# lucidrains/nuwa-pytorch

Hardware: AMD Instinct MI355X
Metric: video-tokens/sec, 3DNA decoder fwd+bwd @ 10x16x16 (higher is better)
Workload: dtype bf16/fp16 operands, fp32 accumulate -- forward: 3-MFMA bf16 hi+lo pairs on cross-attention kv projection, to_logits; 2 fp16 MFMAs (fp16 activation x fp16 hi+lo weight) on to_out x2, cross-attention q projection; single fp16 MFMA on 3DNA q/k/v projection, FF1 + gate, FF2, Sparse3DNA core, cross-atten

## Files before the change

### nuwa_pytorch_amd/csrc/s3_args.h

```cpp
#pragma once
#include <type_traits>
#include "common.h"
#include "../../include/amdnuwa.h"

struct S3Args {
    const bf16_t *q, *k, *v, *ql, *kl, *vl; int ld;
    bf16_t *o, *ol; int ldo;
    int ol_f16;
    const bf16_t *dO, *dOl; int lddo;
    bf16_t *dq, *dk, *dv, *dql, *dkl, *dvl; int ldd;
    const float* wth;
    const float* bias;
    float *ds, *pm;
    float* stats;
    float *part_th, *part_k0, *part_v0;
    float* dwth;
    int B, ntok, F, H, W, kf, kh, kw, df, dh, dw, NH;
    int of, oh, ow;
    int xmode, FK, kvrows, kvoff, ldk, lddk;
    const bf16_t *k0, *k0l, *v0, *v0l; long long k0_bs;
    const uint8_t* kmask;
    float *dnull_k, *dnull_v;
    float scale;
    int accumulate;
    int dbg;
    int ymajor;
    int sep_passes;
    int packed;
    const float* gs2;
    int NT, TW, SW;
};

struct S3DropArgs : S3Args { const uint8_t* keep; float drop_s; };
template <bool DROP> struct S3KArgsSel { using type = S3Args; };
template <> struct S3KArgsSel<true> { using type = S3DropArgs; };
template <bool DROP> using S3KArgs = typename S3KArgsSel<DROP>::type;
template <bool DROP> inline S3KArgs<DROP> s3_kargs(const S3Args& a, const uint8_t* keep, float drop_s) {
    if constexpr (DROP) {
        S3DropArgs d{};
        static_cast<S3Args&>(d) = a;
        d.keep = keep; d.drop_s = drop_s;
        return d;
    } else {
        return a;
    }
}

struct S3Tile { int tw, nt, sw; };
// ... 108 lines not shown
```

### nuwa_pytorch_amd/csrc/sparse3dna.hip

```cpp
#include <cmath>
#include "common.h"
#include "s3_args.h"

namespace {

constexpr int KHMAX = 3;

struct PlaneIt { int ta, tb, fr, yr; };

template <int CH, typename Fn>
__device__ __forceinline__ void sweep_taps(const S3Args& a, const bf16_t* src, const bf16_t* srcl, int b, int f, int y, int w,
                                           int h, int c, bool act, bool qvalid, bf16_t* st_hi, Fn&& fn) {
    const int HS = a.W * a.NH * 32;
    bf16_t* st_lo = st_hi + (CH / 8) * HS;
    const int myslot = ((w * a.NH + h) * 4 + c) * 8;
    const int yr0 = y - a.oh * a.dh;
    uint4 rh[CH / 8], rl[CH / 8];
    auto seek = [&](PlaneIt& p) {
        while (p.ta < a.kf && !(p.fr >= 0 && p.yr >= 0 && p.fr < a.FK && p.yr < a.H)) {
            ++p.tb; p.yr += a.dh;
            if (p.tb == a.kh) { p.tb = 0; p.yr = yr0; ++p.ta; p.fr += a.df; }
        }
    };
    auto step = [&](PlaneIt& p) {
// ... 490 lines not shown
                else {
                    const size_t ci = (((size_t)b * nq + pq) * J + 1 + slot_plane(tp) * a.kw + tc) * a.NH + h;
                    dsv = a.ds[ci]; pmv = a.pm[ci];
                }
                const int slot = ((wq * a.NH + h) * 4 + c) * 8;
                if (LO) {
                    float qq[CH], dd[CH];
                    load_chunk<CH>(sq_hi + slot, a.ql ? sq_lo + slot : nullptr, qq, HS);
                    load_chunk<CH>(sd_hi + slot, a.dOl ? sd_lo + slot : nullptr, dd, HS);
#pragma unroll
                    for (int e = 0; e < CH; ++e) { dkf[e] += dsv * qq[e]; dvf[e] += pmv * dd[e]; }
                } else {
                    uint32_t qk2[CH / 2], dk2[CH / 2];
                    load_pk<CH>(sq_hi + slot, qk2, HS);
                    load_pk<CH>(sd_hi + slot, dk2, HS);
                    axpy_pk<CH>(dkf, dsv, qk2);
                    axpy_pk<CH>(dvf, pmv, dk2);
                }
            }
        }
        tp = tn;
    }
    if (kvalid) {
#pragma unroll
        for (int e = 0; e < CH; ++e) dkf[e] *= a.scale;
        const size_t g = ((size_t)b * a.kvrows + ik) * a.lddk + h * DH + c * CH;
        store_chunk<CH>(a.dk + g, a.dkl ? a.dkl + g : nullptr, dkf);
        store_chunk<CH>(a.dv + g, a.dvl ? a.dvl + g : nullptr, dvf);
    }
}

__global__ __launch_bounds__(1024) void s3_bwd_fin_kernel(S3Args a, int DH) {
    __shared__ float red[2][16][64];
    const int rows = a.F * a.H * a.NT, inner = a.NH * DH;
    const int lane = threadIdx.x & 63, rg = threadIdx.x >> 6;
    const int nchunk = (inner + 63) / 64;
    if ((int)blockIdx.x >= a.B * nchunk) {
        __shared__ float redw[64][17];
        const int nn = a.NH * a.NH;
        const int col = (blockIdx.x - a.B * nchunk) * 16 + (threadIdx.x & 15), rg64 = threadIdx.x >> 4;
        float s = 0.f;
        if (col < nn) {
            const int n = a.B * rows;
            for (int k = rg64; k < n; k += 64 * 8) {
                float v[8];
#pragma unroll
                for (int u = 0; u < 8; ++u) {
                    const int ku = k + 64 * u;
                    const float t = a.part_th[(size_t)(ku < n ? ku : 0) * nn + col];
                    v[u] = ku < n ? t : 0.f;
                }
#pragma unroll
                for (int u = 0; u < 8; ++u) s += v[u];
            }
        }
        redw[rg64][threadIdx.x & 15] = s;
        __syncthreads();
        if (rg64 == 0 && col < nn) {
            float t = 0.f;
#pragma unroll
            for (int r = 0; r < 64; ++r) t += redw[r][threadIdx.x & 15];
            t *= f16_gs_inv(a.gs2);
            a.dwth[col] = a.accumulate ? a.dwth[col] + t : t;
        }
        return;
    }
    if (a.xmode) {
// ... 116 lines not shown
        y = cl + (ii / a.F) * a.dh; f = ii % a.F;
        return;
    }
    y = r2 / a.F; f = r2 % a.F;
}
constexpr int S3M_PAD = 4;
__device__ __forceinline__ int s3m_ts(int J) { return J * S3M_NH + S3M_PAD; }
__device__ __forceinline__ int s3m_item(int item, float rJ) { return item * S3M_NH + (int)(((float)item + 0.5f) * rJ) * S3M_PAD; }

#ifndef S3_MIX_PIN
#define S3_MIX_PIN 0
#endif
#if S3_MIX_PIN
#define S3_MIX_PIN_ASM(s) asm volatile("" : "+v"(s))
#else
#define S3_MIX_PIN_ASM(s) ((void)0)
#endif
__device__ __forceinline__ void lds_store8_done(float* p, const float (&v)[8]) {
#if S3_MIX_PIN
    __builtin_amdgcn_sched_barrier(0);
#endif
#pragma unroll
    for (int g = 0; g < 8; ++g) p[g] = v[g];
#if S3_MIX_PIN
    asm volatile("s_waitcnt lgkmcnt(0)" ::: "memory");
    __builtin_amdgcn_sched_barrier(0);
#endif
}

__device__ __forceinline__ uint2 s3m_keep8(const uint8_t* keep, size_t item) { return *reinterpret_cast<const uint2*>(keep + item * S3M_NH); }
__device__ __forceinline__ bool s3m_kept(uint2 m, int g) { return (((g < 4 ? m.x : m.y) >> (8 * (g & 3))) & 0xffu) != 0u; }
__device__ __forceinline__ bool s3m_kept(uint32_t m, int g) { return ((m >> (8 * g)) & 0xffu) != 0u; }

__device__ __forceinline__ void rowm_planes(const S3Args& a, int f, int y, int* pslot, int* ptok) {
    const int ta0 = max(0, a.kf - 1 - f / a.df), tb0 = max(0, a.kh - 1 - y / a.dh);
    const int nb = a.kh - tb0, n = (a.kf - ta0) * nb;
    const int e = threadIdx.x;
    if (e < n) {
        const int ta = ta0 + e / nb, tb = tb0 + e % nb;
        pslot[e] = 1 + (ta * a.kh + tb) * a.kw;
        ptok[e] = 1 + ((f - (a.kf - 1 - ta) * a.df) * a.H + (y - (a.kh - 1 - tb) * a.dh)) * S3M_W;
    }
    if (e == 0) pslot[S3M_PLANES] = n;
    __syncthreads();
}
__device__ __forceinline__ RowM rowm_init(const S3Args& a, int b, int ry, const int* pslot, const int* ptok) {
    RowM r;
    r.nplanes = pslot[S3M_PLANES];
    r.J = a.kf * a.kh * a.kw + 1;
    r.TS = s3m_ts(r.J);
    r.lane = threadIdx.x & 63; r.wave = threadIdx.x >> 6; r.c = r.lane & 15; r.g4 = r.lane >> 4;
    r.tok0 = (size_t)b * a.ntok;
    r.iq = 1 + ry * S3M_W + r.c;
    r.qok = r.iq < a.ntok;
    r.pslot = pslot; r.ptok = ptok;
    r.vps = r.lane < r.nplanes ? pslot[r.lane] : 0;
    r.vpt = r.lane < r.nplanes ? ptok[r.lane] : 0;
#pragma unroll
    for (int q = 0; q < 4; ++q) {
        const int d = r.c - (4 * r.g4 + q);
        r.tsel[q] = -1;
#pragma unroll
        for (int tc = 0; tc < S3M_KW; ++tc)
            if (tc < a.kw && d == (a.kw - 1 - tc) * a.dw) r.tsel[q] = tc;
    }
    return r;
}

__device__ __forceinline__ void mfma_band_scores(const S3Args& a, const RowM& r, const bf16_t* rows, int ldr, const bf16_t* frag,
                                                 int ldf, int h, float* TAB, float mul, const float* bias) {
    constexpr int NH = S3M_NH, DH = S3M_DH;
    const bf16_t* qrow = frag + (r.tok0 + r.iq) * ldf + h * DH + r.g4 * 8;
    const bf16x8 qf0 = ldg8(qrow, r.qok), qf1 = ldg8(qrow + 32, r.qok);
    const bf16_t* kbase = rows + r.tok0 * ldr + h * DH + r.g4 * 8;
    const int spb = r.c * r.TS + h;
    int sidx[4];
#pragma unroll
    for (int q = 0; q < 4; ++q) sidx[q] = spb + (r.tsel[q] < 0 ? 0 : r.tsel[q]) * NH;
    constexpr int PF = S3M_PF;
    bf16x8 kq0[PF], kq1[PF];
    auto issue = [&](int sq, bf16x8& d0, bf16x8& d1) {
        if (sq > r.nplanes) { d0 = d1 = bf16x8{}; return; }
        const int tok = sq == 0 ? 0 : r.ptok[sq - 1] + r.c;
        const bf16_t* kp = kbase + (size_t)tok * ldr;
// ... 275 lines not shown
            d0 = base + r8 < a.ntok ? ldg_u4(sb, so + v0) : make_uint4(0, 0, 0, 0);
            d1 = base + r8 + 8 < a.ntok ? ldg_u4(sb, so + v1) : make_uint4(0, 0, 0, 0);
        }
    };
    fetch2(0, st[0], st[1]); fetch2(1, st[2], st[3]);
    for (int pi = 0; pi < r.nplanes; pi += 2) {
#pragma unroll
        for (int i = 0; i < 4; ++i) *reinterpret_cast<uint4*>(tile + woff[i]) = st[i];
        const unsigned jb0 = 4u * NH * (unsigned)__builtin_amdgcn_readlane(r.vps, pi);
        const bool two = pi + 1 < r.nplanes;
        const unsigned jb1 = two ? 4u * NH * (unsigned)__builtin_amdgcn_readlane(r.vps, pi + 1) : jb0;
        if (pi + 2 < r.nplanes) { fetch2(pi + 2, st[0], st[1]); fetch2(pi + 3, st[2], st[3]); }
        float pf[8];
#pragma unroll
        for (int j = 0; j < 4; ++j) {
            const float x0 = lds_ld32(sidx4[j] + jb0), x1 = lds_ld32(sidx4[j] + jb1);
            pf[j] = on[j] ? x0 : 0.f;
            pf[4 + j] = (on[j] && two) ? x1 : 0.f;
        }
        const bf16x8 pb = __builtin_bit_cast(bf16x8, make_uint4(pack2_t<F16>(pf[0], pf[1]), pack2_t<F16>(pf[2], pf[3]),
                                                                 pack2_t<F16>(pf[4], pf[5]), pack2_t<F16>(pf[6], pf[7])));
        __builtin_amdgcn_wave_barrier();
#pragma unroll
        for (int db = 0; db < 4; ++db) {
            const s16x4 lo = __builtin_amdgcn_ds_read_tr16_b64_v4i16((lds_s16x4_t*)(tile + troff[db]));
            const s16x4 hi = __builtin_amdgcn_ds_read_tr16_b64_v4i16((lds_s16x4_t*)(tile + troff[db] + 2048));
            const s16x8 v8 = {lo[0], lo[1], lo[2], lo[3], hi[0], hi[1], hi[2], hi[3]};
            O[db] = mfma16<F16>(__builtin_bit_cast(bf16x8, v8), pb, O[db]);
        }
        __builtin_amdgcn_wave_barrier();
    }
}

__device__ __forceinline__ void rowm_softmax(float* TAB, int J, float* gst = nullptr, int wvalid = 0, float pre = 1.f) {
    constexpr int NH = S3M_NH;
    const int t = threadIdx.x, cc = t & 3, wh = t >> 2, h = wh % NH, w = wh / NH;
    TAB += w * s3m_ts(J) + h;
    if (J <= 48) {
        float v[12];
#pragma unroll
        for (int k = 0; k < 12; ++k) { const int j = cc + 4 * k; v[k] = j < J ? TAB[j * NH] * pre : NEG_MAX; }
        float m = NEG_MAX;
#pragma unroll
        for (int k = 0; k < 12; ++k) m = fmaxf(m, v[k]);
        m = quad_max(m);
        float sum = 0.f;
#pragma unroll
        for (int k = 0; k < 12; ++k) {
            const float e = cc + 4 * k < J ? __expf(v[k] - m) : 0.f;
            v[k] = e;
            if (cc + 4 * k < J) sum += e;
        }
        sum = quad_sum(sum);
        const float inv = 1.f / sum;
#pragma unroll
        for (int k = 0; k < 12; ++k) { const int j = cc + 4 * k; if (j < J) TAB[j * NH] = v[k] * inv; }
        if (gst && cc == 0 && w < wvalid) *reinterpret_cast<float2*>(gst + (w * NH + h) * 4) = make_float2(m, inv);
        return;
    }
    float m = NEG_MAX;
    for (int j = cc; j < J; j += 4) m = fmaxf(m, TAB[j * NH] * pre);
    m = quad_max(m);
    float sum = 0.f;
    for (int j = cc; j < J; j += 4) {
        const int idx = j * NH;
        const float e = __expf(TAB[idx] * pre - m);
        TAB[idx] = e;
        sum += e;
    }
// ... 579 lines not shown
    __syncthreads();
    {
        const int g = r.wave;
        f32x4 O[ROWS][4];
        if (!(a.dbg & 4)) {
            if (r.nk <= 64) tile_band_apply_fast<ROWS, F16>(a, r, a.v, a.ld, g, SP, vt_base + r.wave * 4096, O);
            else tile_band_apply<ROWS, F16>(a, r, a.v, a.ld, g, SP, vt_base + r.wave * 4096, O);
        }
        else {
#pragma unroll
            for (int i = 0; i < ROWS; ++i)
#pragma unroll
                for (int db = 0; db < 4; ++db) O[i][db] = f32x4{0.f, 0.f, 0.f, 0.f};
        }
#pragma unroll
        for (int i = 0; i < ROWS; ++i) {
            if (!r.qok[i]) continue;
            const size_t go = (r.tok0 + r.iq[i]) * a.ldo + g * DH + 4 * r.g4;
#pragma unroll
            for (int db = 0; db < 4; ++db) {
                const uint32_t h01 = pack2_rne(O[i][db][0], O[i][db][1]), h23 = pack2_rne(O[i][db][2], O[i][db][3]);
                if (!F16 || a.o) *reinterpret_cast<uint2*>(a.o + go + db * 16) = make_uint2(h01, h23);
                if (F16 && a.ol)
                    *reinterpret_cast<uint2*>(a.ol + go + db * 16) = a.ol_f16 ?
                        make_uint2(pack2_f16_sat(O[i][db][0], O[i][db][1]), pack2_f16_sat(O[i][db][2], O[i][db][3])) :
                        make_uint2(pack2_rne(O[i][db][0] - lo_f(h01), O[i][db][1] - hi_f(h01)), pack2_rne(O[i][db][2] - lo_f(h23), O[i][db][3] - hi_f(h23)));
            }
        }
    }
}

typedef _Float16 f16x4_t __attribute__((ext_vector_type(4)));
constexpr float S3Q_DPS = 0.015625f;
template <bool BIAS, bool G16 = false, bool DROP = false>
__global__ __launch_bounds__(512, 4) void s3_bwd_q_mfma_kernel(S3KArgs<DROP> a) {
    constexpr int NH = S3M_NH, DH = S3M_DH, W = S3M_W, inner = NH * DH;
    extern __shared__ __attribute__((aligned(16))) char smem[];
    const int J = a.kf * a.kh * a.kw + 1, TS = s3m_ts(J), nsp = W * TS;
    const float rJ = 1.f / (float)J;
    const size_t r1 = (size_t)nsp * 4 > 8 * 4096 ? (size_t)nsp * 4 : 8 * 4096;
    float* SP = reinterpret_cast<float*>(smem);
    float* DP = reinterpret_cast<float*>(smem + r1);
    float* RED = DP + nsp;
    float* PM0 = RED + 8 * 64;
    __shared__ float wsh[64];
    __shared__ int pslot[S3M_PLANES + 1], ptok[S3M_PLANES + 1];
    const int t = threadIdx.x;
    const int rows = a.F * a.H;
    const int bid = xcd_row_id();
    const int b = bid / rows, r2 = bid % rows;
    int f, y;
    s3m_row_order(a, r2, f, y);
    const int ry = f * a.H + y;
    const int nq = a.ntok - 1;
    if (t < NH * NH) wsh[t] = a.wth[t];
    float* pth = a.part_th + (size_t)bid * NH * NH;
    float* pk0 = a.part_k0 + (size_t)bid * inner;
    float* pv0 = a.part_v0 + (size_t)bid * inner;
    if (ry == 0)
        for (int e = t; e < inner; e += blockDim.x) a.dq[((size_t)b * a.ntok) * a.ldd + e] = 0;
    if (ry * W + 1 >= a.ntok) {
        for (int e = t; e < NH * NH; e += blockDim.x) pth[e] = 0.f;
        for (int e = t; e < inner; e += blockDim.x) { pk0[e] = 0.f; pv0[e] = 0.f; }
        return;
    }
    {
        const float4 neg4 = make_float4(NEG_MAX, NEG_MAX, NEG_MAX, NEG_MAX), zero4 = make_float4(0.f, 0.f, 0.f, 0.f);
        for (int e = t; e < nsp / 4 && !(a.dbg & 2048); e += blockDim.x) { reinterpret_cast<float4*>(SP)[e] = neg4; reinterpret_cast<float4*>(DP)[e] = zero4; }
    }
    rowm_planes(a, f, y, pslot, ptok);
    const RowM r = rowm_init(a, b, ry, pslot, ptok);
    char* stile = reinterpret_cast<char*>(PM0 + W * NH) + r.wave * 2048;
    if (!(a.dbg & 1)) {
    if constexpr (!BIAS) {
    mfma_band_scores_fast<G16>(a, r, a.k, a.ld, a.q, a.ld, r.wave, SP, 1.f, stile);
    mfma_band_scores_fast<G16>(a, r, a.v, a.ld, a.dO, a.lddo, r.wave, DP, G16 ? S3Q_DPS : 1.f, stile);
    } else {
    mfma_band_scores_staged<G16>(a, r, a.k, a.ld, a.q, a.ld, r.wave, SP, BIAS ? a.scale : 1.f, BIAS ? a.bias : nullptr, stile);
    mfma_band_scores_staged<G16>(a, r, a.v, a.ld, a.dO, a.lddo, r.wave, DP, G16 ? S3Q_DPS : 1.f, nullptr, stile);
    }
    }
    __syncthreads();
    float* gst = a.stats ? a.stats + ((size_t)b * nq + (size_t)ry * W) * NH * 4 : nullptr;
    const int wvalid = a.ntok - 1 - ry * W;
    if (!(a.dbg & 64)) rowm_softmax(SP, J, gst, wvalid, BIAS ? 1.f : a.scale);
    [[maybe_unused]] float dps_back = 1.f / S3Q_DPS;
    if constexpr (DROP) {
        dps_back *= a.drop_s;
        const float sdp = G16 ? 1.f : a.drop_s;
        for (int item = t; item < W * J; item += blockDim.x) {
            const int wq = (int)(((float)item + 0.5f) * rJ), iq = 1 + ry * W + wq;
            if (iq < a.ntok) {
                const uint2 m = s3m_keep8(a.keep, ((size_t)b * nq + (iq - 1)) * J + (item - wq * J));
                const int ib = item * NH + wq * S3M_PAD;
                float4 d0 = *reinterpret_cast<const float4*>(DP + ib), d1 = *reinterpret_cast<const float4*>(DP + ib + 4);
                d0.x = s3m_kept(m, 0) ? d0.x * sdp : 0.f; d0.y = s3m_kept(m, 1) ? d0.y * sdp : 0.f;
                d0.z = s3m_kept(m, 2) ? d0.z * sdp : 0.f; d0.w = s3m_kept(m, 3) ? d0.w * sdp : 0.f;
                d1.x = s3m_kept(m, 4) ? d1.x * sdp : 0.f; d1.y = s3m_kept(m, 5) ? d1.y * sdp : 0.f;
                d1.z = s3m_kept(m, 6) ? d1.z * sdp : 0.f; d1.w = s3m_kept(m, 7) ? d1.w * sdp : 0.f;
                *reinterpret_cast<float4*>(DP + ib) = d0;
                *reinterpret_cast<float4*>(DP + ib + 4) = d1;
            }
        }
    }
    __syncthreads();
    if constexpr (G16) {
        const int lane = t & 63, wv = t >> 6, n16 = lane & 15, kg = lane >> 4, sset = n16 >> 3, kh = kg & 1;
        const bool on = (n16 < 8) == (kg < 2);
        f16x4_t awt_hi, awt_lo;
#pragma unroll
        for (int i = 0; i < 4; ++i) {
            const float wt = on ? wsh[(4 * kh + i) * NH + (n16 & 7)] : 0.f;
            const _Float16 h16 = (_Float16)wt;
            awt_hi[i] = h16; awt_lo[i] = (_Float16)(wt - (float)h16);
        }
        const int nitems = W * J, ngrp = (nitems + 31) >> 5;
        f32x4 CW = {0.f, 0.f, 0.f, 0.f};
        float dp_amax = 0.f;
        for (int G = wv; G < ngrp && !(a.dbg & 128); G += 8) {
            {
                const int ib0 = 32 * G + 16 * sset + 4 * kg;
                float avf[4], bvf[4];
#pragma unroll
                for (int ts = 0; ts < 4; ++ts) {
                    const int item = ib0 + ((ts + sset + 2 * kh) & 3);
                    const bool ok = item < nitems;
                    const int idx = s3m_item(ok ? item : 0, rJ) + (n16 & 7);
                    avf[ts] = ok ? DP[idx] : 0.f;
                    bvf[ts] = ok ? SP[idx] : 0.f;
                }
                const f16x4_t av = __builtin_bit_cast(f16x4_t, make_uint2(pack2_f16_sat(avf[0], avf[1]), pack2_f16_sat(avf[2], avf[3])));
                const f16x4_t bv = __builtin_bit_cast(f16x4_t, make_uint2(pack2_f16(bvf[0], bvf[1]), pack2_f16(bvf[2], bvf[3])));
                CW = __builtin_amdgcn_mfma_f32_16x16x16f16(av, bv, CW, 0, 0, 0);
            }
            const int item = 32 * G + 16 * (kg >> 1) + n16;
            const bool ok = item < nitems;
            const int ib = s3m_item(ok ? item : 0, rJ) + 4 * kh;
            const float4 d4 = *reinterpret_cast<const float4*>(DP + ib);
            const f16x4_t df = __builtin_bit_cast(f16x4_t, make_uint2(pack2_f16_sat_n(d4.x, d4.y, dp_amax), pack2_f16_sat_n(d4.z, d4.w, dp_amax)));
            f32x4 rr = {0.f, 0.f, 0.f, 0.f};
            rr = __builtin_amdgcn_mfma_f32_16x16x16f16(awt_hi, df, rr, 0, 0, 0);
            rr = __builtin_amdgcn_mfma_f32_16x16x16f16(awt_lo, df, rr, 0, 0, 0);
            if (ok) *reinterpret_cast<float4*>(DP + ib) = make_float4(rr[0], rr[1], rr[2], rr[3]);
        }
        f16_sat_commit(dp_amax);
        float tw[4];
#pragma unroll
        for (int i = 0; i < 4; ++i) tw[i] = CW[i] + __shfl(CW[i], (lane + 40) & 63, 64);
        if (n16 < 8 && kg < 2) {
#pragma unroll
            for (int i = 0; i < 4; ++i) RED[wv * 64 + (4 * kg + i) * NH + n16] = tw[i] * dps_back;
        }
        __syncthreads();
        if (t < NH * NH) {
            float sum = 0.f;
            for (int k = 0; k < 8; ++k) sum += RED[k * 64 + t];
            pth[t] = sum;
        }
        __syncthreads();
    } else if (!a.sep_passes) {
        float red_lane = 0.f;
#pragma unroll
        for (int half = 0; half < 2; ++half) {
            float acc[32];
#pragma unroll
            for (int k = 0; k < 32; ++k) acc[k] = 0.f;
#pragma unroll 1
            for (int item = t; item < W * J && !(a.dbg & 128); item += blockDim.x) {
                const int wq = (int)(((float)item + 0.5f) * rJ), j = item - wq * J;
                const int iq = 1 + ry * W + wq;
                const int ib = item * NH + wq * S3M_PAD;
                const float4 p0 = *reinterpret_cast<const float4*>(SP + ib), p1 = *reinterpret_cast<const float4*>(SP + ib + 4);
                const float4 d0 = *reinterpret_cast<const float4*>(DP + ib), d1 = *reinterpret_cast<const float4*>(DP + ib + 4);
                const float pv[8] = {p0.x, p0.y, p0.z, p0.w, p1.x, p1.y, p1.z, p1.w};
                const float dv_[8] = {d0.x, d0.y, d0.z, d0.w, d1.x, d1.y, d1.z, d1.w};
                const float* wv = wsh;
                asm volatile("" : "+v"(wv));
                float res[8];
#pragma unroll
                for (int x = 0; x < 8; ++x) res[x] = 0.f;
#pragma unroll
                for (int g = 0; g < 8; ++g) {
                    const float4 w0 = *reinterpret_cast<const float4*>(wv + g * NH), w1 = *reinterpret_cast<const float4*>(wv + g * NH + 4);
                    const float wg[8] = {w0.x, w0.y, w0.z, w0.w, w1.x, w1.y, w1.z, w1.w};
                    if (half == 0) {
                        if (!a.packed) {
                            float sm = 0.f;
#pragma unroll
                            for (int hh = 0; hh < 8; ++hh) sm += wg[hh] * pv[hh];
                            res[g] = sm;
                        }
// ... 8 lines not shown
                }
                if (half == 0) {
                    if (!a.packed) {
                        if constexpr (DROP) {
                            if (iq < a.ntok) {
                                const uint2 m = s3m_keep8(a.keep, ((size_t)b * nq + (iq - 1)) * J + j);
#pragma unroll
                                for (int g = 0; g < 8; ++g) res[g] = s3m_kept(m, g) ? res[g] * a.drop_s : 0.f;
                            }
                        }
                        if (iq < a.ntok && !gst && !(a.dbg & 2)) {
                            float4* dst = reinterpret_cast<float4*>(a.pm + (((size_t)b * nq + (iq - 1)) * J + j) * NH);
                            dst[0] = make_float4(res[0], res[1], res[2], res[3]);
                            dst[1] = make_float4(res[4], res[5], res[6], res[7]);
                        }
                        if (j == 0) {
#pragma unroll
                            for (int g = 0; g < 8; ++g) PM0[wq * NH + g] = iq < a.ntok ? res[g] : 0.f;
                        }
                    }
                } else {
                    *reinterpret_cast<float4*>(DP + ib) = make_float4(res[0], res[1], res[2], res[3]);
                    *reinterpret_cast<float4*>(DP + ib + 4) = make_float4(res[4], res[5], res[6], res[7]);
                }
            }
            const int lane = t & 63;
#pragma unroll
            for (int off = 16, cnt = 16; off >= 1; off >>= 1, cnt >>= 1) {
                const bool upper = (lane & off) != 0;
#pragma unroll
                for (int i = 0; i < cnt; ++i) {
                    const float send = upper ? acc[i] : acc[i + cnt];
                    const float keep = upper ? acc[i + cnt] : acc[i];
                    acc[i] = keep + __shfl_xor(send, off, 64);
                }
            }
            const float tot = acc[0] + __shfl_xor(acc[0], 32, 64);
            if ((lane >> 5) == half) red_lane = tot;
        }
        RED[(t >> 6) * 64 + (t & 63)] = red_lane;
        __syncthreads();
        if (t < NH * NH) {
            float s = 0.f;
            for (int k = 0; k < 8; ++k) s += RED[k * 64 + t];
            pth[t] = s;
        }
        __syncthreads();
    } else {
        float wr[64];
#pragma unroll
        for (int k = 0; k < 64; ++k) wr[k] = wsh[k];
        for (int item0 = t; item0 < (gst ? W : W * J); item0 += blockDim.x) {
            const int item = gst ? item0 * J : item0;
            const int wq = (int)(((float)item + 0.5f) * rJ), j = item - wq * J;
            const int iq = 1 + ry * W + wq;
            float pv[8];
    #pragma unroll
            for (int hh = 0; hh < 8; ++hh) pv[hh] = SP[item * NH + wq * S3M_PAD + hh];
            float* dst = a.pm + (((size_t)b * nq + (iq - 1)) * J + j) * NH;
            [[maybe_unused]] uint2 km = make_uint2(0u, 0u);
            if constexpr (DROP) { if (iq < a.ntok) km = s3m_keep8(a.keep, ((size_t)b * nq + (iq - 1)) * J + j); }
    #pragma unroll
            for (int g = 0; g < 8; ++g) {
                float s = 0.f;
    #pragma unroll
                for (int hh = 0; hh < 8; ++hh) s += wr[g * NH + hh] * pv[hh];
                if constexpr (DROP) s = s3m_kept(km, g) ? s * a.drop_s : 0.f;
                if (iq < a.ntok && !gst && !(a.dbg & 2)) dst[g] = s;
                if (j == 0) PM0[wq * NH + g] = iq < a.ntok ? s : 0.f;
            }
        }
        {
            const int pair = t & 63, grp = t >> 6;
            const int g = pair / NH, hh = pair % NH;
            float acc = 0.f;
            for (int item = grp; item < W * J && !(a.dbg & 8); item += 8 * 8) {
                float dv8[8], pv8[8];
    #pragma unroll
                for (int u = 0; u < 8; ++u) {
                    const int it = item + 8 * u, itc = it < W * J ? it : grp;
                    const int ib = s3m_item(itc, rJ);
                    dv8[u] = DP[ib + g]; pv8[u] = SP[ib + hh];
                }
    #pragma unroll
                for (int u = 0; u < 8; ++u) acc += item + 8 * u < W * J ? dv8[u] * pv8[u] : 0.f;
            }
            RED[grp * 64 + pair] = acc;
            __syncthreads();
            if (t < NH * NH) {
                float s = 0.f;
                for (int k = 0; k < 8; ++k) s += RED[k * 64 + t];
                pth[t] = s;
            }
            __syncthreads();
        }
        for (int item = t; item < W * J; item += blockDim.x) {
            float dv_[8], out[8];
            const int ib = s3m_item(item, rJ);
    #pragma unroll
            for (int g = 0; g < 8; ++g) dv_[g] = DP[ib + g];
    #pragma unroll
            for (int hh = 0; hh < 8; ++hh) {
                float s = 0.f;
    #pragma unroll
                for (int g = 0; g < 8; ++g) s += wr[g * NH + hh] * dv_[g];
                S3_MIX_PIN_ASM(s);
                out[hh] = s;
            }
            lds_store8_done(DP + ib, out);
        }
        __syncthreads();
    }
    {
        const int cc = t & 3, wh = t >> 2, h = wh % NH, w = wh / NH;
        const int i = 1 + ry * W + w;
        float ds_amax = 0.f;
        if (a.dbg & 256) {
        } else if (J <= 48) {
            float pv[12], dv[12];
#pragma unroll
            for (int k = 0; k < 12; ++k) {
                const int j = cc + 4 * k, idx = w * TS + (j < J ? j : cc) * NH + h;
                pv[k] = SP[idx]; dv[k] = DP[idx];
            }
            float d = 0.f;
#pragma unroll
            for (int k = 0; k < 12; ++k) if (cc + 4 * k < J) d += pv[k] * dv[k];
            d = quad_sum(d);
            if (gst && cc == 0 && i < a.ntok) gst[(w * NH + h) * 4 + 2] = d;
#pragma unroll
            for (int k = 0; k < 12; ++k) {
                const int j = cc + 4 * k;
                if (j < J) {
                    const int idx = w * TS + j * NH + h;
                    float dsv = pv[k] * (dv[k] - d);
                    if constexpr (G16) { dsv *= dps_back; ds_amax = fmaxf(ds_amax, fabsf(dsv)); dsv = f16_clamp(dsv); }
                    DP[idx] = dsv;
                    if (i < a.ntok && !gst && !a.packed && !(a.dbg & 2)) a.ds[(((size_t)b * nq + (i - 1)) * J + j) * NH + h] = dsv;
                }
            }
        } else {
        float d = 0.f;
        for (int j = cc; j < J; j += 4) d += SP[w * TS + j * NH + h] * DP[w * TS + j * NH + h];
        d = quad_sum(d);
// ... 119 lines not shown
        const int eg = t & 63, wv = t >> 6, h = eg >> 3;
        float sk[8], sv[8];
#pragma unroll
        for (int k = 0; k < 8; ++k) { sk[k] = 0.f; sv[k] = 0.f; }
        uint4 qv[2], dv4[2];
        float cs[2], cp[2];
#pragma unroll
        for (int rr = 0; rr < 2; ++rr) {
            const int w = 2 * wv + rr, i = 1 + ry * W + w;
            const bool in = i < a.ntok;
            const size_t ic = r.tok0 + (in ? i : a.ntok - 1);
            qv[rr] = *reinterpret_cast<const uint4*>(a.q + ic * a.ld + 8 * eg);
            dv4[rr] = *reinterpret_cast<const uint4*>(a.dO + ic * a.lddo + 8 * eg);
            cs[rr] = in ? DP[w * TS + h] : 0.f;
            cp[rr] = in ? PM0[w * NH + h] : 0.f;
        }
#pragma unroll
        for (int rr = 0; rr < 2; ++rr) {
            const uint32_t qw[4] = {qv[rr].x, qv[rr].y, qv[rr].z, qv[rr].w}, dw[4] = {dv4[rr].x, dv4[rr].y, dv4[rr].z, dv4[rr].w};
#pragma unroll
            for (int k = 0; k < 4; ++k) {
                sk[2 * k] = fmaf(cs[rr], lo_t<G16>(qw[k]), sk[2 * k]); sk[2 * k + 1] = fmaf(cs[rr], hi_t<G16>(qw[k]), sk[2 * k + 1]);
                sv[2 * k] = fmaf(cp[rr], lo_t<G16>(dw[k]), sv[2 * k]); sv[2 * k + 1] = fmaf(cp[rr], hi_t<G16>(dw[k]), sv[2 * k + 1]);
            }
        }
        float4* dst = reinterpret_cast<float4*>(part + (wv * 64 + eg) * 16);
        const int rot = eg >> 2;
        dst[rot & 3] = make_float4(sk[0], sk[1], sk[2], sk[3]); dst[(1 + rot) & 3] = make_float4(sk[4], sk[5], sk[6], sk[7]);
        dst[(2 + rot) & 3] = make_float4(sv[0], sv[1], sv[2], sv[3]); dst[(3 + rot) & 3] = make_float4(sv[4], sv[5], sv[6], sv[7]);
    }
    __syncthreads();
    if (!(a.dbg & 1024)) {
        const float* part = reinterpret_cast<const float*>(smem);
        for (int e = t; e < inner; e += blockDim.x) {
            const int eg = e >> 3, cmp = e & 7, rot = eg >> 2;
            const int ok_ = 4 * (((cmp >> 2) + rot) & 3) + (cmp & 3), ov_ = 4 * ((2 + (cmp >> 2) + rot) & 3) + (cmp & 3);
            float sk = 0.f, sv = 0.f;
#pragma unroll
            for (int wv = 0; wv < 8; ++wv) {
                sk += part[(wv * 64 + eg) * 16 + ok_];
                sv += part[(wv * 64 + eg) * 16 + ov_];
            }
            pk0[e] = a.scale * sk;
            pv0[e] = sv;
        }
    }
}

template <bool PACKED, bool G16 = false>
__global__ __launch_bounds__(512, 2) void s3_bwd_kv_mfma_kernel(S3Args a) {
    constexpr int NH = S3M_NH, DH = S3M_DH, W = S3M_W;
    extern __shared__ __attribute__((aligned(16))) char smem[];
    __shared__ int pslot[S3M_PLANES + 1], ptok[S3M_PLANES + 1];
    const int t = threadIdx.x, lane = t & 63, wave = t >> 6, c = lane & 15, g4 = lane >> 4, h = wave;
    const int rows = a.F * a.H;
    const int bid = xcd_row_id();
    const int b = bid / rows, r2 = bid % rows;
    int f, y;
    s3m_row_order(a, r2, f, y);
    const int ry = f * a.H + y;
    const int J = a.kf * a.kh * a.kw + 1, nq = a.ntok - 1;
    if (ry * W + 1 >= a.ntok) return;
    if (t < 64) {
        const int ta = t / a.kh, tb = t % a.kh;
        const int fq = f + (a.kf - 1 - ta) * a.df, yq = y + (a.kh - 1 - tb) * a.dh;
        const bool ok = t < a.kf * a.kh && fq < a.F && yq < a.H && (fq * a.H + yq) * W + 1 < a.ntok;
        const unsigned long long m = __ballot(ok);
        if (ok) {
            const int pos = __popcll(m & ((1ull << t) - 1ull));
            pslot[pos] = 1 + (ta * a.kh + tb) * a.kw; ptok[pos] = 1 + (fq * a.H + yq) * W;
        }
        if (t == 0) pslot[S3M_PLANES] = __popcll(m);
    }
    __syncthreads();
    const int nplanes = pslot[S3M_PLANES];
    const size_t tok0 = (size_t)b * a.ntok;
    int tsel[4];
#pragma unroll
    for (int j = 0; j < 4; ++j) {
// ... 304 lines not shown
        __builtin_amdgcn_wave_barrier();
    }
    if (kok) {
        bf16_t* kr = a.dk + (tok0 + ik) * a.ldd + h * DH + 4 * g4;
        bf16_t* vr = a.dv + (tok0 + ik) * a.ldd + h * DH + 4 * g4;
        float amax = 0.f;
#pragma unroll
        for (int db = 0; db < 4; ++db) {
            if constexpr (G16) {
                *reinterpret_cast<uint2*>(kr + db * 16) = make_uint2(pack2_f16_sat_n(dK[db][0] * a.scale, dK[db][1] * a.scale, amax),
                                                                     pack2_f16_sat_n(dK[db][2] * a.scale, dK[db][3] * a.scale, amax));
                *reinterpret_cast<uint2*>(vr + db * 16) = make_uint2(pack2_f16_sat_n(dV[db][0], dV[db][1], amax), pack2_f16_sat_n(dV[db][2], dV[db][3], amax));
            } else {
                *reinterpret_cast<uint2*>(kr + db * 16) = make_uint2(pack2_rne(dK[db][0] * a.scale, dK[db][1] * a.scale),
                                                                     pack2_rne(dK[db][2] * a.scale, dK[db][3] * a.scale));
                *reinterpret_cast<uint2*>(vr + db * 16) = make_uint2(pack2_rne(dV[db][0], dV[db][1]), pack2_rne(dV[db][2], dV[db][3]));
            }
        }
        if constexpr (G16) f16_sat_commit(amax);
    }
}


bool s3_mfma_geom(const amdnuwa_s3_geom* g) {
    return !g->noncausal && g->W == 16 && g->heads == 8 && g->dim_head == 64 && g->kw <= S3M_KW && g->kf * g->kh <= S3M_PLANES;
}
int s3_tile_rows(const amdnuwa_s3_geom* g, int want) {
    if (want == 0) want = S3T_AUTO_ROWS;
    for (int rws = want >= 4 ? 4 : (want >= 2 ? 2 : 1); rws > 1; rws >>= 1)
        if (g->dh > 0 && g->H % (g->dh * rws) == 0 && g->kf * (g->kh + rws - 1) <= S3T_MAXK) return rws;
    return 1;
}

enum : int { S3K_FWD = 3,
             S3K_BWD = 4,
             S3K_TILE_ROWS = 16,
             S3K_SEP_PASSES = 19,
             S3K_WS_FP32 = 24,
             S3K_DROP_VALU = 26 };
enum S3Form { S3_BF16, S3_HILO, S3_F16 };
enum S3KvSide { S3KV_VALU, S3KV_BAND_F32, S3KV_BAND_PACKED, S3KV_BAND_RC };
struct S3Route {
    bool f16;
    bool fwd_band; int tile_rows;
    bool q_band; S3KvSide kv;
    int packed, sep_passes, ymajor;
};
S3Route s3_route(const amdnuwa_s3_geom* g, S3Form form, bool masked, bool cross = false) {
    const int* t = g_amdnuwa_tuning;
    S3Route r{};
    r.tile_rows = 1;
    r.ymajor = (t[S3K_FWD] & 2) ? 0 : 1;
    if (cross) return r;
    if (form == S3_F16) {
        r.f16 = r.fwd_band = r.q_band = true; r.kv = S3KV_BAND_PACKED; r.packed = 1;
    } else {
        const bool band = form == S3_BF16 && s3_mfma_geom(g) && !(masked && t[S3K_DROP_VALU] == 1);
        r.fwd_band = band && !(t[S3K_FWD] & 1);
        r.q_band = band && t[S3K_BWD] != 1;
        const bool kv_band = r.q_band && t[S3K_BWD] != 2;
        r.sep_passes = t[S3K_SEP_PASSES] == 1;
        r.packed = (kv_band && !g->d_rel_bias && t[S3K_WS_FP32] != 1 && !r.sep_passes) ? 1 : 0;
        r.kv = !kv_band ? S3KV_VALU : (t[S3K_BWD] == 4 && !g->d_rel_bias && !masked) ? S3KV_BAND_RC : r.packed ? S3KV_BAND_PACKED : S3KV_BAND_F32;
    }
    if (r.fwd_band) r.tile_rows = s3_tile_rows(g, t[S3K_TILE_ROWS]);
    return r;
}

void fill_geom(S3Args& a, const amdnuwa_s3_geom* g, const S3Route& r) {
    a.B = g->B; a.ntok = g->ntok; a.F = g->F; a.H = g->H; a.W = g->W; a.kf = g->kf; a.kh = g->kh; a.kw = g->kw;
    a.df = g->df; a.dh = g->dh; a.dw = g->dw; a.NH = g->heads; a.scale = g->scale; a.bias = g->rel_bias;
    a.ymajor = r.ymajor;
    a.of = g->noncausal ? (g->kf - 1) / 2 : g->kf - 1;
    a.oh = g->noncausal ? (g->kh - 1) / 2 : g->kh - 1;
    a.ow = g->noncausal ? (g->kw - 1) / 2 : g->kw - 1;
    a.xmode = 0; a.FK = g->F; a.kvrows = g->ntok; a.kvoff = 1; a.kmask = nullptr;
    const S3Tile tl = s3_tile(g);
    a.NT = tl.nt; a.TW = tl.tw; a.SW = tl.sw;
}
void self_kv(S3Args& a) {
    a.ldk = a.ld; a.lddk = a.ldd;
    a.k0 = a.k; a.k0l = a.kl; a.v0 = a.v; a.v0l = a.vl; a.k0_bs = (long long)a.ntok * a.ld;
}
int block_threads(const amdnuwa_s3_geom* g) { return ((g->W * g->heads * 4 + 63) / 64) * 64; }

struct S3Ws { size_t ds, pm, part_th, part_k0, part_v0, colsum, bytes; };
S3Ws s3_ws(const amdnuwa_s3_geom* g) {
    const size_t nq = g->ntok - 1, items = (size_t)g->B * nq * s3_slots(g) * g->heads;
    const size_t parts = (size_t)g->B * g->F * g->H * s3_tile(g).nt, inner = (size_t)g->heads * g->dim_head;
    S3Ws w{};
    w.pm = items; w.part_th = 2 * items; w.part_k0 = w.part_th + parts * g->heads * g->heads; w.part_v0 = w.part_k0 + parts * inner;
    w.colsum = w.part_v0 + parts * inner;
    w.bytes = w.colsum * sizeof(float) + 256 + amdnuwa_colsum_workspace_bytes((long long)g->B * nq, (int)(s3_slots(g) * g->heads));
    return w;
}
S3Ws bind_ws(S3Args& a, const amdnuwa_s3_geom* g, void* workspace) {
    const S3Ws w = s3_ws(g);
    float* ws = (float*)workspace;
    a.ds = ws + w.ds; a.pm = ws + w.pm; a.part_th = ws + w.part_th; a.part_k0 = ws + w.part_k0; a.part_v0 = ws + w.part_v0;
    return w;
}

struct S3Mask { bool on; const uint8_t* keep; float s; };
bool keep_aligned(const uint8_t* keep) { return (reinterpret_cast<uintptr_t>(keep) & 7u) == 0; }
bool mask_ok(const S3Mask& m, bool band) { return !m.on || (m.keep && std::isfinite(m.s) && m.s >= 1.f && (!band || keep_aligned(m.keep))); }

int s3_fwd_launch(const S3Args& a, const amdnuwa_s3_geom* g, const S3Route& r, bool lo, const uint8_t* keep, float drop_s, hipStream_t stream) {
    if (!r.fwd_band) {
        const size_t lds = s3_lds(g, lo).fwd;
        if (a.NT > 1) return s3w_fwd_launch(a, g->dim_head, lo, lds, keep, drop_s, stream);
        return s3_dispatch(g->dim_head, lo, keep != nullptr, [&](auto dh, auto lo_c, auto dr) {
            return s3_launch(s3_fwd_kernel<dh(), lo_c(), dr()>, dim3(g->B * g->F * g->H), dim3(block_threads(g)), lds, stream, s3_kargs<dr()>(a, keep, drop_s));
        });
    }
    const int tr = r.tile_rows;
    const size_t lm = (size_t)tr * 16 * (s3_slots(g) * 8 + 4) * sizeof(float) + 8 * 4096;
    const dim3 grid(g->B * g->F * (g->H / tr)), block(512);
    return s3_if(r.f16, [&](auto f16) { return s3_if(keep != nullptr, [&](auto dr) {
        const auto ka = s3_kargs<dr()>(a, keep, drop_s);
        if (tr == 1) return s3_launch(s3_fwd_mfma_kernel<f16(), dr()>, grid, block, lm, stream, ka);
        return s3_if(a.bias != nullptr, [&](auto bias) {
            return tr == 4 ? s3_launch(s3_fwd_tile_kernel<4, f16(), bias(), dr()>, grid, block, lm, stream, ka)
                           : s3_launch(s3_fwd_tile_kernel<2, f16(), bias(), dr()>, grid, block, lm, stream, ka);
        });
    }); });
}

int s3_bwd_launch(const S3Args& a, const amdnuwa_s3_geom* g, const S3Route& r, bool lo, const uint8_t* keep, float drop_s, hipStream_t stream) {
    const S3Lds l = s3_lds(g, lo);
    int rc;
    if (a.NT > 1) {
        rc = s3w_bwd_launch(a, g->dim_head, lo, l.bq, l.bkv, keep, drop_s, stream);
    } else {
        const dim3 grid_q(g->B * g->F * g->H), grid_kv(g->B * a.FK * g->H), block(block_threads(g)), band(512);
        if (r.q_band) {
            const size_t nspm = (size_t)g->W * (s3_slots(g) * g->heads + 4);
            const size_t lds_qm = (nspm * 4 > 8 * 4096 ? nspm * 4 : 8 * 4096) + nspm * 4 + (8 * 64 + 16 * 8) * 4 + 8 * 2048;
            rc = s3_if(keep != nullptr, [&](auto dr) {
                const auto ka = s3_kargs<dr()>(a, keep, drop_s);
                if (r.f16) return s3_launch(s3_bwd_q_mfma_kernel<false, true, dr()>, grid_q, band, lds_qm, stream, ka);
                return s3_if(a.bias != nullptr, [&](auto bias) { return s3_launch(s3_bwd_q_mfma_kernel<bias(), false, dr()>, grid_q, band, lds_qm, stream, ka); });
            });
        } else {
            rc = s3_dispatch(g->dim_head, lo, keep != nullptr, [&](auto dh, auto lo_c, auto dr) {
                return s3_launch(s3_bwd_q_kernel<dh(), lo_c(), dr()>, grid_q, block, l.bq, stream, s3_kargs<dr()>(a, keep, drop_s));
            });
        }
        if (rc) return rc;
        switch (r.kv) {
        case S3KV_BAND_RC: rc = s3_launch(s3_bwd_kv_rc_mfma_kernel, grid_q, band, 8 * 4096 + 16384, stream, a); break;
        case S3KV_BAND_PACKED:
            rc = r.f16 ? s3_launch(s3_bwd_kv_mfma_kernel<true, true>, grid_q, band, 8 * 8192, stream, a)
                       : s3_launch(s3_bwd_kv_mfma_kernel<true>, grid_q, band, 8 * 8192, stream, a);
            break;
        case S3KV_BAND_F32: rc = s3_launch(s3_bwd_kv_mfma_kernel<false>, grid_q, band, 8 * 8192, stream, a); break;
        case S3KV_VALU:
            rc = s3_dispatch(g->dim_head, lo, false, [&](auto dh, auto lo_c, auto) {
                return s3_launch(s3_bwd_kv_kernel<dh(), lo_c()>, grid_kv, block, l.bkv, stream, a);
            });
        }
    }
    if (rc) return rc;
    hipLaunchKernelGGL(s3_bwd_fin_kernel, dim3(g->B * ((g->heads * g->dim_head + 63) / 64) + (g->heads * g->heads + 15) / 16), dim3(1024), 0, stream, a, g->dim_head);
    LAUNCH_CHECK();
    return AMDNUWA_OK;
}

}

extern "C" int amdnuwa_s3_supported(const amdnuwa_s3_geom* g, int lo_operands) {
    if (check_geom(g)) return 0;
    return s3_lds_need(g, lo_operands != 0) <= S3_LDS_MAX ? 1 : 0;
}
extern "C" int amdnuwa_s3_drop_supported(const amdnuwa_s3_geom* g, int lo_operands) { return amdnuwa_s3_supported(g, lo_operands) && !g->noncausal ? 1 : 0; }
// ... 269 lines not shown
```

Measured before the change: 726,100.

## Let each sparse-3DNA backward-q block process several rows, carrying partial sums

Splits the band backward-q kernel body into a per-row device function and wraps it in a loop so one block can handle several (f,y) rows. The theta, k0 and v0 partials are carried in registers across rows, and the partial buffers and their final reduction shrink by the rows-per-block factor. The default rows-per-block is 1, so by default the work and partition match the old code. A tuning knob selects larger counts and a strided row order.

```diff
diff --git a/nuwa_pytorch_amd/csrc/s3_args.h b/nuwa_pytorch_amd/csrc/s3_args.h
--- a/nuwa_pytorch_amd/csrc/s3_args.h
+++ b/nuwa_pytorch_amd/csrc/s3_args.h
@@ -14,6 +14,8 @@
     float *ds, *pm;
     float* stats;
     float *part_th, *part_k0, *part_v0;
+    int rpw;
+    int rgroups, rstep;
     float* dwth;
     int B, ntok, F, H, W, kf, kh, kw, df, dh, dw, NH;
     int of, oh, ow;
diff --git a/nuwa_pytorch_amd/csrc/sparse3dna.hip b/nuwa_pytorch_amd/csrc/sparse3dna.hip
--- a/nuwa_pytorch_amd/csrc/sparse3dna.hip
+++ b/nuwa_pytorch_amd/csrc/sparse3dna.hip
@@ -546,7 +546,7 @@
 
 __global__ __launch_bounds__(1024) void s3_bwd_fin_kernel(S3Args a, int DH) {
     __shared__ float red[2][16][64];
-    const int rows = a.F * a.H * a.NT, inner = a.NH * DH;
+    const int rows = a.F * a.H * a.NT / a.rpw, inner = a.NH * DH;
     const int lane = threadIdx.x & 63, rg = threadIdx.x >> 6;
     const int nchunk = (inner + 63) / 64;
     if ((int)blockIdx.x >= a.B * nchunk) {
@@ -729,10 +729,10 @@
 __device__ __forceinline__ bool s3m_kept(uint2 m, int g) { return (((g < 4 ? m.x : m.y) >> (8 * (g & 3))) & 0xffu) != 0u; }
 __device__ __forceinline__ bool s3m_kept(uint32_t m, int g) { return ((m >> (8 * g)) & 0xffu) != 0u; }
 
-__device__ __forceinline__ void rowm_planes(const S3Args& a, int f, int y, int* pslot, int* ptok) {
+__device__ __forceinline__ void rowm_planes(const S3Args& a, int f, int y, int* pslot, int* ptok, int tid = threadIdx.x) {
     const int ta0 = max(0, a.kf - 1 - f / a.df), tb0 = max(0, a.kh - 1 - y / a.dh);
     const int nb = a.kh - tb0, n = (a.kf - ta0) * nb;
-    const int e = threadIdx.x;
+    const int e = tid;
     if (e < n) {
         const int ta = ta0 + e / nb, tb = tb0 + e % nb;
         pslot[e] = 1 + (ta * a.kh + tb) * a.kw;
@@ -741,12 +741,12 @@
     if (e == 0) pslot[S3M_PLANES] = n;
     __syncthreads();
 }
-__device__ __forceinline__ RowM rowm_init(const S3Args& a, int b, int ry, const int* pslot, const int* ptok) {
+__device__ __forceinline__ RowM rowm_init(const S3Args& a, int b, int ry, const int* pslot, const int* ptok, int tid = threadIdx.x) {
     RowM r;
     r.nplanes = pslot[S3M_PLANES];
     r.J = a.kf * a.kh * a.kw + 1;
     r.TS = s3m_ts(r.J);
-    r.lane = threadIdx.x & 63; r.wave = threadIdx.x >> 6; r.c = r.lane & 15; r.g4 = r.lane >> 4;
+    r.lane = tid & 63; r.wave = tid >> 6; r.c = r.lane & 15; r.g4 = r.lane >> 4;
     r.tok0 = (size_t)b * a.ntok;
     r.iq = 1 + ry * S3M_W + r.c;
     r.qok = r.iq < a.ntok;
@@ -1088,9 +1088,9 @@
     }
 }
 
-__device__ __forceinline__ void rowm_softmax(float* TAB, int J, float* gst = nullptr, int wvalid = 0, float pre = 1.f) {
+__device__ __forceinline__ void rowm_softmax(float* TAB, int J, float* gst = nullptr, int wvalid = 0, float pre = 1.f, int tid = threadIdx.x) {
     constexpr int NH = S3M_NH;
-    const int t = threadIdx.x, cc = t & 3, wh = t >> 2, h = wh % NH, w = wh / NH;
+    const int t = tid, cc = t & 3, wh = t >> 2, h = wh % NH, w = wh / NH;
     TAB += w * s3m_ts(J) + h;
     if (J <= 48) {
         float v[12];
@@ -1736,44 +1736,40 @@
 
 typedef _Float16 f16x4_t __attribute__((ext_vector_type(4)));
 constexpr float S3Q_DPS = 0.015625f;
-template <bool BIAS, bool G16 = false, bool DROP = false>
-__global__ __launch_bounds__(512, 4) void s3_bwd_q_mfma_kernel(S3KArgs<DROP> a) {
+__device__ __forceinline__ float lane_xor(float v, int lane, int off) {
+    return __builtin_bit_cast(float, __builtin_amdgcn_ds_bpermute((lane ^ off) << 2, __builtin_bit_cast(int, v)));
+}
+struct S3QCarry {
+    f32x4 cw;
+    float th;
+    float k0, v0;
+};
+template <bool BIAS, bool G16, bool DROP>
+__device__ __forceinline__ void s3q_row(const S3KArgs<DROP>& a, int b, int f, int y, char* smem, const float* wsh, int* pslot, int* ptok, S3QCarry& cy) {
     constexpr int NH = S3M_NH, DH = S3M_DH, W = S3M_W, inner = NH * DH;
-    extern __shared__ __attribute__((aligned(16))) char smem[];
-    const int J = a.kf * a.kh * a.kw + 1, TS = s3m_ts(J), nsp = W * TS;
+    static_assert(inner == 512, "thread e of the 512 carries channel e of the <bos> sums");
+    const int J = a.kf * a.kh * a.kw + 1;
+    const int TS = s3m_ts(J), nsp = W * TS;
     const float rJ = 1.f / (float)J;
     const size_t r1 = (size_t)nsp * 4 > 8 * 4096 ? (size_t)nsp * 4 : 8 * 4096;
     float* SP = reinterpret_cast<float*>(smem);
     float* DP = reinterpret_cast<float*>(smem + r1);
-    float* RED = DP + nsp;
-    float* PM0 = RED + 8 * 64;
-    __shared__ float wsh[64];
-    __shared__ int pslot[S3M_PLANES + 1], ptok[S3M_PLANES + 1];
-    const int t = threadIdx.x;
-    const int rows = a.F * a.H;
-    const int bid = xcd_row_id();
-    const int b = bid / rows, r2 = bid % rows;
-    int f, y;
-    s3m_row_order(a, r2, f, y);
+    float* PM0 = DP + nsp + 8 * 64;
+    int t = threadIdx.x;
+    asm volatile("" : "+v"(t));
     const int ry = f * a.H + y;
     const int nq = a.ntok - 1;
-    if (t < NH * NH) wsh[t] = a.wth[t];
-    float* pth = a.part_th + (size_t)bid * NH * NH;
-    float* pk0 = a.part_k0 + (size_t)bid * inner;
-    float* pv0 = a.part_v0 + (size_t)bid * inner;
     if (ry == 0)
         for (int e = t; e < inner; e += blockDim.x) a.dq[((size_t)b * a.ntok) * a.ldd + e] = 0;
-    if (ry * W + 1 >= a.ntok) {
-        for (int e = t; e < NH * NH; e += blockDim.x) pth[e] = 0.f;
-        for (int e = t; e < inner; e += blockDim.x) { pk0[e] = 0.f; pv0[e] = 0.f; }
-        return;
-    }
+    if (ry * W + 1 >= a.ntok) return;
     {
-        const float4 neg4 = make_float4(NEG_MAX, NEG_MAX, NEG_MAX, NEG_MAX), zero4 = make_float4(0.f, 0.f, 0.f, 0.f);
+        float negm = NEG_MAX, zero = 0.f;
+        asm volatile("" : "+v"(negm), "+v"(zero));
+        const float4 neg4 = make_float4(negm, negm, negm, negm), zero4 = make_float4(zero, zero, zero, zero);
         for (int e = t; e < nsp / 4 && !(a.dbg & 2048); e += blockDim.x) { reinterpret_cast<float4*>(SP)[e] = neg4; reinterpret_cast<float4*>(DP)[e] = zero4; }
     }
-    rowm_planes(a, f, y, pslot, ptok);
-    const RowM r = rowm_init(a, b, ry, pslot, ptok);
+    rowm_planes(a, f, y, pslot, ptok, t);
+    RowM r = rowm_init(a, b, ry, pslot, ptok, t);
     char* stile = reinterpret_cast<char*>(PM0 + W * NH) + r.wave * 2048;
     if (!(a.dbg & 1)) {
     if constexpr (!BIAS) {
@@ -1787,7 +1783,7 @@
     __syncthreads();
     float* gst = a.stats ? a.stats + ((size_t)b * nq + (size_t)ry * W) * NH * 4 : nullptr;
     const int wvalid = a.ntok - 1 - ry * W;
-    if (!(a.dbg & 64)) rowm_softmax(SP, J, gst, wvalid, BIAS ? 1.f : a.scale);
+    if (!(a.dbg & 64)) rowm_softmax(SP, J, gst, wvalid, BIAS ? 1.f : a.scale, t);
     [[maybe_unused]] float dps_back = 1.f / S3Q_DPS;
     if constexpr (DROP) {
         dps_back *= a.drop_s;
@@ -1819,7 +1815,7 @@
             awt_hi[i] = h16; awt_lo[i] = (_Float16)(wt - (float)h16);
         }
         const int nitems = W * J, ngrp = (nitems + 31) >> 5;
-        f32x4 CW = {0.f, 0.f, 0.f, 0.f};
+        f32x4& CW = cy.cw;
         float dp_amax = 0.f;
         for (int G = wv; G < ngrp && !(a.dbg & 128); G += 8) {
             {
@@ -1848,19 +1844,6 @@
             if (ok) *reinterpret_cast<float4*>(DP + ib) = make_float4(rr[0], rr[1], rr[2], rr[3]);
         }
         f16_sat_commit(dp_amax);
-        float tw[4];
-#pragma unroll
-        for (int i = 0; i < 4; ++i) tw[i] = CW[i] + __shfl(CW[i], (lane + 40) & 63, 64);
-        if (n16 < 8 && kg < 2) {
-#pragma unroll
-            for (int i = 0; i < 4; ++i) RED[wv * 64 + (4 * kg + i) * NH + n16] = tw[i] * dps_back;
-        }
-        __syncthreads();
-        if (t < NH * NH) {
-            float sum = 0.f;
-            for (int k = 0; k < 8; ++k) sum += RED[k * 64 + t];
-            pth[t] = sum;
-        }
         __syncthreads();
     } else if (!a.sep_passes) {
         float red_lane = 0.f;
@@ -1935,19 +1918,13 @@
                 for (int i = 0; i < cnt; ++i) {
                     const float send = upper ? acc[i] : acc[i + cnt];
                     const float keep = upper ? acc[i + cnt] : acc[i];
-                    acc[i] = keep + __shfl_xor(send, off, 64);
+                    acc[i] = keep + lane_xor(send, lane, off);
                 }
             }
-            const float tot = acc[0] + __shfl_xor(acc[0], 32, 64);
+            const float tot = acc[0] + lane_xor(acc[0], lane, 32);
             if ((lane >> 5) == half) red_lane = tot;
         }
-        RED[(t >> 6) * 64 + (t & 63)] = red_lane;
-        __syncthreads();
-        if (t < NH * NH) {
-            float s = 0.f;
-            for (int k = 0; k < 8; ++k) s += RED[k * 64 + t];
-            pth[t] = s;
-        }
+        cy.th += red_lane;
         __syncthreads();
     } else {
         float wr[64];
@@ -1988,13 +1965,7 @@
     #pragma unroll
                 for (int u = 0; u < 8; ++u) acc += item + 8 * u < W * J ? dv8[u] * pv8[u] : 0.f;
             }
-            RED[grp * 64 + pair] = acc;
-            __syncthreads();
-            if (t < NH * NH) {
-                float s = 0.f;
-                for (int k = 0; k < 8; ++k) s += RED[k * 64 + t];
-                pth[t] = s;
-            }
+            cy.th += acc;
             __syncthreads();
         }
         for (int item = t; item < W * J; item += blockDim.x) {
@@ -2013,6 +1984,11 @@
             lds_store8_done(DP + ib, out);
         }
         __syncthreads();
+    }
+    if constexpr (!G16) {
+        int tr = threadIdx.x;
+        asm volatile("" : "+v"(tr));
+        r = rowm_init(a, b, ry, pslot, ptok, tr);
     }
     {
         const int cc = t & 3, wh = t >> 2, h = wh % NH, w = wh / NH;
@@ -2198,19 +2174,73 @@
     __syncthreads();
     if (!(a.dbg & 1024)) {
         const float* part = reinterpret_cast<const float*>(smem);
-        for (int e = t; e < inner; e += blockDim.x) {
-            const int eg = e >> 3, cmp = e & 7, rot = eg >> 2;
-            const int ok_ = 4 * (((cmp >> 2) + rot) & 3) + (cmp & 3), ov_ = 4 * ((2 + (cmp >> 2) + rot) & 3) + (cmp & 3);
-            float sk = 0.f, sv = 0.f;
-#pragma unroll
-            for (int wv = 0; wv < 8; ++wv) {
-                sk += part[(wv * 64 + eg) * 16 + ok_];
-                sv += part[(wv * 64 + eg) * 16 + ov_];
-            }
-            pk0[e] = a.scale * sk;
-            pv0[e] = sv;
-        }
-    }
+        const int e = t, eg = e >> 3, cmp = e & 7, rot = eg >> 2;
+        const int ok_ = 4 * (((cmp >> 2) + rot) & 3) + (cmp & 3), ov_ = 4 * ((2 + (cmp >> 2) + rot) & 3) + (cmp & 3);
+        float sk = 0.f, sv = 0.f;
+#pragma unroll
+        for (int wv = 0; wv < 8; ++wv) {
+            sk += part[(wv * 64 + eg) * 16 + ok_];
+            sv += part[(wv * 64 + eg) * 16 + ov_];
+        }
+        cy.k0 += a.scale * sk;
+        cy.v0 += sv;
+    }
+}
+
+template <bool BIAS, bool G16 = false, bool DROP = false>
+__global__ __launch_bounds__(512, 4) void s3_bwd_q_mfma_kernel(S3KArgs<DROP>) {
+    constexpr int NH = S3M_NH, inner = S3M_NH * S3M_DH;
+    extern __shared__ __attribute__((aligned(16))) char smem[];
+    __shared__ float wsh[64];
+    __shared__ int pslot[S3M_PLANES + 1], ptok[S3M_PLANES + 1];
+    const int t = threadIdx.x;
+    auto args = [] {
+        typedef const __attribute__((address_space(4))) S3KArgs<DROP>* kargs_t;
+        kargs_t kp = (kargs_t)__builtin_amdgcn_kernarg_segment_ptr();
+        asm volatile("" : "+s"(kp));
+        S3KArgs<DROP> r;
+        __builtin_memcpy(&r, kp, sizeof(r));
+        return r;
+    };
+    S3KArgs<DROP> ar = args();
+    const int rpw = ar.rpw, groups = ar.rgroups, rstep = ar.rstep;
+    const int bid = xcd_row_id();
+    const int b = bid / groups, r2_0 = (bid % groups) * (rstep == 1 ? rpw : 1);
+    if (t < NH * NH) wsh[t] = ar.wth[t];
+    S3QCarry cy{f32x4{0.f, 0.f, 0.f, 0.f}, 0.f, 0.f, 0.f};
+    for (int i = 0; i < rpw; ++i) {
+        int f, y;
+        s3m_row_order(ar, r2_0 + i * rstep, f, y);
+        s3q_row<BIAS, G16, DROP>(ar, b, f, y, smem, wsh, pslot, ptok, cy);
+        if (i + 1 < rpw) {
+            __syncthreads();
+            ar = args();
+        }
+    }
+    const int nsp = S3M_W * s3m_ts(ar.kf * ar.kh * ar.kw + 1);
+    float* RED = reinterpret_cast<float*>(smem + ((size_t)nsp * 4 > 8 * 4096 ? (size_t)nsp * 4 : 8 * 4096)) + nsp;
+    if constexpr (G16) {
+        const int lane = t & 63, wv = t >> 6, n16 = lane & 15, kg = lane >> 4;
+        float dps_back = 1.f / S3Q_DPS;
+        if constexpr (DROP) dps_back *= ar.drop_s;
+        float tw[4];
+#pragma unroll
+        for (int k = 0; k < 4; ++k) tw[k] = cy.cw[k] + __shfl(cy.cw[k], (lane + 40) & 63, 64);
+        if (n16 < 8 && kg < 2) {
+#pragma unroll
+            for (int k = 0; k < 4; ++k) RED[wv * 64 + (4 * kg + k) * NH + n16] = tw[k] * dps_back;
+        }
+    } else {
+        RED[t] = cy.th;
+    }
+    __syncthreads();
+    if (t < NH * NH) {
+        float sum = 0.f;
+        for (int k = 0; k < 8; ++k) sum += RED[k * 64 + t];
+        ar.part_th[(size_t)bid * NH * NH + t] = sum;
+    }
+    ar.part_k0[(size_t)bid * inner + t] = cy.k0;
+    ar.part_v0[(size_t)bid * inner + t] = cy.v0;
 }
 
 template <bool PACKED, bool G16 = false>
@@ -2581,9 +2611,17 @@
     return 1;
 }
 
+constexpr int S3Q_AUTO_RPW = 1;
+int s3_bwd_rpw(const amdnuwa_s3_geom* g, int want) {
+    int rpw = 1;
+    while (rpw * 2 <= (want > 0 ? want : S3Q_AUTO_RPW) && (g->F * g->H) % (rpw * 2) == 0) rpw *= 2;
+    return rpw;
+}
+
 enum : int { S3K_FWD = 3,
              S3K_BWD = 4,
              S3K_TILE_ROWS = 16,
+             S3K_BWD_RPW = 18,
              S3K_SEP_PASSES = 19,
              S3K_WS_FP32 = 24,
              S3K_DROP_VALU = 26 };
@@ -2594,11 +2632,12 @@
     bool fwd_band; int tile_rows;
     bool q_band; S3KvSide kv;
     int packed, sep_passes, ymajor;
+    int rpw, rstep;
 };
 S3Route s3_route(const amdnuwa_s3_geom* g, S3Form form, bool masked, bool cross = false) {
     const int* t = g_amdnuwa_tuning;
     S3Route r{};
-    r.tile_rows = 1;
+    r.tile_rows = r.rpw = r.rstep = 1;
     r.ymajor = (t[S3K_FWD] & 2) ? 0 : 1;
     if (cross) return r;
     if (form == S3_F16) {
@@ -2613,13 +2652,14 @@
         r.kv = !kv_band ? S3KV_VALU : (t[S3K_BWD] == 4 && !g->d_rel_bias && !masked) ? S3KV_BAND_RC : r.packed ? S3KV_BAND_PACKED : S3KV_BAND_F32;
     }
     if (r.fwd_band) r.tile_rows = s3_tile_rows(g, t[S3K_TILE_ROWS]);
+    if (r.q_band) { r.rpw = s3_bwd_rpw(g, t[S3K_BWD_RPW] & 255); r.rstep = (t[S3K_BWD_RPW] & 256) ? g->F * g->H / r.rpw : 1; }
     return r;
 }
 
 void fill_geom(S3Args& a, const amdnuwa_s3_geom* g, const S3Route& r) {
     a.B = g->B; a.ntok = g->ntok; a.F = g->F; a.H = g->H; a.W = g->W; a.kf = g->kf; a.kh = g->kh; a.kw = g->kw;
     a.df = g->df; a.dh = g->dh; a.dw = g->dw; a.NH = g->heads; a.scale = g->scale; a.bias = g->rel_bias;
-    a.ymajor = r.ymajor;
+    a.ymajor = r.ymajor; a.rpw = r.rpw; a.rstep = r.rstep; a.rgroups = g->F * g->H / r.rpw;
     a.of = g->noncausal ? (g->kf - 1) / 2 : g->kf - 1;
     a.oh = g->noncausal ? (g->kh - 1) / 2 : g->kh - 1;
     a.ow = g->noncausal ? (g->kw - 1) / 2 : g->kw - 1;
@@ -2681,14 +2721,14 @@
     if (a.NT > 1) {
         rc = s3w_bwd_launch(a, g->dim_head, lo, l.bq, l.bkv, keep, drop_s, stream);
     } else {
-        const dim3 grid_q(g->B * g->F * g->H), grid_kv(g->B * a.FK * g->H), block(block_threads(g)), band(512);
+        const dim3 grid_q(g->B * g->F * g->H), grid_qw(g->B * (g->F * g->H / r.rpw)), grid_kv(g->B * a.FK * g->H), block(block_threads(g)), band(512);
         if (r.q_band) {
             const size_t nspm = (size_t)g->W * (s3_slots(g) * g->heads + 4);
             const size_t lds_qm = (nspm * 4 > 8 * 4096 ? nspm * 4 : 8 * 4096) + nspm * 4 + (8 * 64 + 16 * 8) * 4 + 8 * 2048;
             rc = s3_if(keep != nullptr, [&](auto dr) {
                 const auto ka = s3_kargs<dr()>(a, keep, drop_s);
-                if (r.f16) return s3_launch(s3_bwd_q_mfma_kernel<false, true, dr()>, grid_q, band, lds_qm, stream, ka);
-                return s3_if(a.bias != nullptr, [&](auto bias) { return s3_launch(s3_bwd_q_mfma_kernel<bias(), false, dr()>, grid_q, band, lds_qm, stream, ka); });
+                if (r.f16) return s3_launch(s3_bwd_q_mfma_kernel<false, true, dr()>, grid_qw, band, lds_qm, stream, ka);
+                return s3_if(a.bias != nullptr, [&](auto bias) { return s3_launch(s3_bwd_q_mfma_kernel<bias(), false, dr()>, grid_qw, band, lds_qm, stream, ka); });
             });
         } else {
             rc = s3_dispatch(g->dim_head, lo, keep != nullptr, [&](auto dh, auto lo_c, auto dr) {
```

Result: no change. 727,300, median of 3 (+0.2%).
